# IIT-PAVIS/Acoustic-Image-Generation

Hardware: AMD Instinct MI355X
Metric: train-step images/sec (higher is better)
Workload: dtype f32

## Files before the change

acoustic-image-generation_amd/csrc/conv_halo16_kernel.hpp:

```cpp
#pragma once
#include "igemm_split3_kernel.hpp"

namespace acimg {

struct ConvHaloParams {
    const float* X; int H, W, ldx;
    const char* Wimg; unsigned w_lo_off;
    const float* a_scale; const float* a_shift; int a_relu;
    float* Y; int ldy, nout;
    const float* bias; const float* res; int ldres; const float* mask; int ldmask;
    float* stats; int stats_ld;
    int tiles_x, tiles_y; long tiles;
};

template <typename TR, int TERMS, int CIN, int NOUT, int MODE>
__global__ __launch_bounds__(512, 1) void conv_halo16_kernel(const ConvHaloParams p) {
    typedef typename TR::V8 V8;
    constexpr int TH = TERMS == 1 ? 8 : 4, TW = 32, XH = TH + 2, XWV = TW + 2, XW = 36;
    constexpr int PITCH = CIN * 2 + 16;
    constexpr int XPL = XH * XW * PITCH;
    constexpr int KTOT = 9 * CIN;
    constexpr int WROW = KTOT * 2 + 16;
    constexpr int WPL = NOUT * WROW;
    constexpr int NPL = TERMS == 3 ? 2 : 1;
    constexpr int MT = TERMS == 1 ? 2 : 1;
    constexpr int NT = NOUT / 16;
    constexpr int NXL = (XH * XWV * (CIN / 4) + 511) / 512;
    extern __shared__ __attribute__((aligned(16))) float ch16_smem[];
    char* const xl = reinterpret_cast<char*>(ch16_smem);
    char* const wl = xl + NPL * XPL;
    const int tid = threadIdx.x, lane = tid & 63, wid = tid >> 6;
    const int li = lane & 15, g = lane >> 4;
    const int jrow = TERMS == 1 ? wid : wid >> 1;
    const int mcol0 = TERMS == 1 ? 0 : (wid & 1) * 16;

    for (int i = tid; i < NPL * NOUT * (KTOT / 8); i += 512) {
        const int ch = i % (KTOT / 8), r2 = i / (KTOT / 8);
        const int n = r2 % NOUT, pl = r2 / NOUT;
        const uint4 v = *reinterpret_cast<const uint4*>(p.Wimg + (size_t)pl * p.w_lo_off + ((size_t)n * KTOT + ch * 8) * 2);
        *reinterpret_cast<uint4*>(wl + pl * WPL + n * WROW + ch * 16) = v;
    }

    float4 rx[NXL];
    unsigned okm = 0;
    const float4 asc = p.a_scale ? *reinterpret_cast<const float4*>(p.a_scale + (tid % (CIN / 4)) * 4) : make_float4(1.f, 1.f, 1.f, 1.f);
    const float4 ash = p.a_scale ? *reinterpret_cast<const float4*>(p.a_shift + (tid % (CIN / 4)) * 4) : make_float4(0.f, 0.f, 0.f, 0.f);
    auto load_tile = [&](long tile) {
        okm = 0;
        const int tx = (int)(tile % p.tiles_x);
        const long t2 = tile / p.tiles_x;
        const int ty = (int)(t2 % p.tiles_y);
        const long img = t2 / p.tiles_y;
        const float* xi = p.X + img * p.H * p.W * p.ldx;
#pragma unroll
        for (int k = 0; k < NXL; ++k) {
            const int i = tid + 512 * k;
            const int c4 = i % (CIN / 4), pix = i / (CIN / 4);
            const int row = pix / XWV, col = pix - row * XWV;
            const int iy = ty * TH + row - 1, ix = tx * TW + col - 1;
            float4 v = make_float4(0.f, 0.f, 0.f, 0.f);
            if (row < XH && (unsigned)iy < (unsigned)p.H && (unsigned)ix < (unsigned)p.W) {
                v = *reinterpret_cast<const float4*>(xi + ((long)iy * p.W + ix) * p.ldx + c4 * 4);
                okm |= 1u << k;
            }
            rx[k] = v;
        }
    };
    auto store_tile = [&]() {
#pragma unroll
        for (int k = 0; k < NXL; ++k) {
            const int i = tid + 512 * k;
            const int c4 = i % (CIN / 4), pix = i / (CIN / 4);
            const int row = pix / XWV, col = pix - row * XWV;
            if (row < XH) {
                const int off = (row * XW + col) * PITCH + c4 * 8;
                uint2 hi, lo;
                split4<TR>(p.a_scale && ((okm >> k) & 1u) ? affine_relu4(rx[k], asc, ash, p.a_relu != 0) : rx[k], hi, lo);
                *reinterpret_cast<uint2*>(xl + off) = hi;
                if (TERMS == 3) *reinterpret_cast<uint2*>(xl + XPL + off) = lo;
            }
        }
    };

    f32x4 s1[NT], s2[NT];
#pragma unroll
    for (int n = 0; n < NT; ++n) s1[n] = s2[n] = f32x4{0.f, 0.f, 0.f, 0.f};
    f32x4 bv[NT];
#pragma unroll
    for (int n = 0; n < NT; ++n)
        bv[n] = (MODE == 0 && p.bias) ? *reinterpret_cast<const f32x4*>(p.bias + n * 16 + 4 * g) : f32x4{0.f, 0.f, 0.f, 0.f};

    const int a_base = (jrow * XW + mcol0 + li) * PITCH + g * 16;
    const int b_base = li * WROW + g * 16;

    long tile = blockIdx.x;
    if (tile < p.tiles) load_tile(tile);
    for (; tile < p.tiles; tile += gridDim.x) {
        __syncthreads();
        store_tile();
        __syncthreads();
        const int tx = (int)(tile % p.tiles_x);
        const long t2 = tile / p.tiles_x;
        const int ty = (int)(t2 % p.tiles_y);
        const long img = t2 / p.tiles_y;
        if (tile + gridDim.x < p.tiles) load_tile(tile + gridDim.x);
        f32x4 acc[MT][NT];
#pragma unroll
        for (int m = 0; m < MT; ++m)
#pragma unroll
            for (int n = 0; n < NT; ++n) acc[m][n] = f32x4{0.f, 0.f, 0.f, 0.f};
#pragma unroll
        for (int r = 0; r < 3; ++r)
#pragma unroll
            for (int s_ = 0; s_ < 3; ++s_)
#pragma unroll
                for (int ck = 0; ck < CIN / 32; ++ck) {
                    V8 ah[MT], al[MT], bh[NT], bl[NT];
#pragma unroll
                    for (int m = 0; m < MT; ++m) {
                        const int off = a_base + (r * XW + s_ + 16 * m) * PITCH + ck * 64;
                        ah[m] = *reinterpret_cast<const V8*>(xl + off);
                        if (TERMS == 3) al[m] = *reinterpret_cast<const V8*>(xl + XPL + off);
                    }
#pragma unroll
                    for (int n = 0; n < NT; ++n) {
                        const int off = b_base + n * 16 * WROW + ((r * 3 + s_) * CIN + ck * 32) * 2;
                        bh[n] = *reinterpret_cast<const V8*>(wl + off);
                        if (TERMS == 3) bl[n] = *reinterpret_cast<const V8*>(wl + WPL + off);
                    }
#pragma unroll
                    for (int m = 0; m < MT; ++m)
#pragma unroll
                        for (int n = 0; n < NT; ++n) {
                            if (TERMS == 3) {
                                acc[m][n] = TR::mfma(bl[n], ah[m], acc[m][n]);
                                acc[m][n] = TR::mfma(bh[n], al[m], acc[m][n]);
                            }
                            acc[m][n] = TR::mfma(bh[n], ah[m], acc[m][n]);
                        }
                }
        const int oy = ty * TH + jrow;
#pragma unroll
        for (int m = 0; m < MT; ++m) {
            const int ox = tx * TW + mcol0 + 16 * m + li;
            if (oy < p.H && ox < p.W) {
                const long pix = (img * p.H + oy) * p.W + ox;
#pragma unroll
                for (int n = 0; n < NT; ++n) {
                    if (NOUT == 16 && n * 16 + 4 * g >= p.nout) continue;
                    f32x4 v = acc[m][n] * TR::OUTSCALE + bv[n];
                    if (MODE == 1) {
                        if (p.res) v += *reinterpret_cast<const f32x4*>(p.res + pix * p.ldres + n * 16 + 4 * g);
                        if (p.mask) {
                            const f32x4 k = *reinterpret_cast<const f32x4*>(p.mask + pix * p.ldmask + n * 16 + 4 * g);
#pragma unroll
                            for (int c = 0; c < 4; ++c) v[c] = k[c] > 0.f ? v[c] : 0.f;
                        }
                    } else {
                        s1[n] += v;
                        s2[n] += v * v;
                    }
                    *reinterpret_cast<f32x4*>(p.Y + pix * p.ldy + n * 16 + 4 * g) = v;
                }
            }
        }
    }
    if (MODE == 0 && p.stats) {
        __syncthreads();
        float* red = reinterpret_cast<float*>(xl);
#pragma unroll
        for (int n = 0; n < NT; ++n)
#pragma unroll
            for (int c = 0; c < 4; ++c) {
                const float a = row16_sum(s1[n][c]), b = row16_sum(s2[n][c]);
                if (li == 0) {
                    red[(wid * 2 + 0) * NOUT + n * 16 + 4 * g + c] = a;
                    red[(wid * 2 + 1) * NOUT + n * 16 + 4 * g + c] = b;
                }
            }
        __syncthreads();
        if (tid < 2 * NOUT) {
            const int which = tid / NOUT, n = tid % NOUT;
            float t = 0.f;
#pragma unroll
            for (int w = 0; w < 8; ++w) t += red[(w * 2 + which) * NOUT + n];
            p.stats[((long)blockIdx.x * 2 + which) * p.stats_ld + n] = t;
        }
    }
}

static constexpr int CONV_HALO16_WGS = 256;

}
```

acoustic-image-generation_amd/csrc/igemm.hip:

```cpp
#include "wgrad_split3_kernel.hpp"
#include "wgrad_tap_kernel.hpp"
#include "conv_tap_kernel.hpp"
#include "igemm_split3d_kernel.hpp"
#include "igemm_split3dp_kernel.hpp"
#include "igemm_split3r_kernel.hpp"
#include "igemm_split3h_kernel.hpp"
#include "skinny_kernel.hpp"
#include "wgrad_f32_kernel.hpp"
#include "wgrad_halo_kernel.hpp"
#include "direct_conv_kernel.hpp"
#include "conv_few16_kernel.hpp"
#include "patch2_kernel.hpp"
#include "conv_halo16_kernel.hpp"
#include "conv_aux_kernels.hpp"
#include <cstdlib>
#include <algorithm>
#include <type_traits>

namespace acimg {

static void launch_slab_reduce_wide(const float* slab, int splits, long rows, int ncols, int ld, float* out, const float* slab2,
                                    float* out2, hipStream_t st) {
    const long total = rows * ncols;
    if (total <= 4096) {
// ... 138 lines not shown
            return fail(ACIMG_EINVAL, "igemm: ticket words must be 16-byte aligned");
        const bool handoff = tickets != nullptr && tiles <= ACIMG_TICKET_WORDS && g_cfg.splitk_handoff;
        if (handoff) need = (size_t)p.splits * tiles * c.bm * c.bn * sizeof(float);
        if (ws == nullptr || ws_bytes < need)
            return fail(ACIMG_EWORKSPACE, "igemm: workspace %zu < %zu", ws_bytes, need);
        p.slab = static_cast<float*>(ws);
        if (handoff) p.ts_counters = static_cast<int*>(tickets);
    }
    if (c.bm == 128 && c.bn == 128) launch_cfg<128, 128, 2, 4, 512>(p, nt, cal, grid, st);
    else if (c.bm == 128 && c.bn == 64) launch_cfg<128, 64, 2, 2, 256>(p, nt, cal, grid, st);
    else if (c.bm == 64 && c.bn == 64) launch_cfg<64, 64, 2, 2, 256>(p, nt, cal, grid, st);
    else launch_cfg<256, 16, 4, 1, 256>(p, nt, cal, grid, st);
    int rc = check_launch("igemm");
    if (rc) return rc;
    if (p.splits > 1) {
        if (p.ts_counters == nullptr) {
            const long total = (long)p.M * p.Ngemm;
            hipLaunchKernelGGL(igemm_splitk_reduce_kernel, dim3(cdiv(total, 256)), dim3(256), 0, st,
                               p.slab, p.splits, p.M, p.Ngemm, p.slab_ld, p.e);
            rc = check_launch("igemm_splitk_reduce");
        }
        if (!rc && stats_after) {
            hipLaunchKernelGGL(partial_stats_kernel, dim3(cdiv(p.M, 256)), dim3(256), 0, st, e.Y, e.ldy, p.M,
                               e.Nstore, stats_after, e.stats_ld, 256);
            rc = check_launch("partial_stats");
        }
    }
    return rc;
}

static int pick_wgrad_splits(int M, int KK, int Ngemm, int bmo, int bn) {
    const long tiles = (long)cdiv(KK, bmo) * cdiv(Ngemm, bn);
    long s = (512 + tiles - 1) / tiles;
    const int minpix = g_cfg.wgrad_minpix;
    const long maxs = (M + minpix - 1) / minpix;
    long cap = 128;
    if ((long)KK * Ngemm <= 8192) {
        s = (2048 + tiles - 1) / tiles;
        cap = 2048;
    }
    if (s > maxs) s = maxs;
    if (s > cap) s = cap;
    if (s < 1) s = 1;
    return (int)s;
}
static void wgrad_tile(int Ngemm, int& bmo, int& bn) {
    bmo = 128;
    bn = Ngemm <= 16 ? 16 : (Ngemm <= 32 ? 32 : (Ngemm <= 64 ? 64 : 128));
    if (Ngemm > 64 && cdiv(Ngemm, 64) * 64 < cdiv(Ngemm, 128) * 128) bn = 64;
}
static int wgrad_split3_bn(int Ngemm) {
    return Ngemm > 64 ? 128 : (Ngemm > 32 ? 64 : 32);
}
static bool wgrad_halo16_shape(long M, int KK, int Ngemm) { return Ngemm <= 32 && KK % 9 == 0 && KK <= 9 * 64 && M >= 65536; }
static bool wgrad_tap_shape(int KK, int Ngemm) { return KK % 9 == 0 && KK >= 9 * 64 && Ngemm > 32; }
static size_t wgrad_ws_bytes(int M, int KK, int Ngemm, int ldo) {
    int bmo, bn;
    wgrad_tile(Ngemm, bmo, bn);
    int s = std::max(pick_wgrad_splits(M, KK, Ngemm, bmo, bn), pick_wgrad_splits(M, KK, Ngemm, bmo, wgrad_split3_bn(Ngemm)));
    if (wgrad_halo16_shape(M, KK, Ngemm) && s < (KK <= 9 * 16 ? 512 : 256)) s = KK <= 9 * 16 ? 512 : 256;
    return s > 1 ? (size_t)(s + 1) * ((size_t)KK + 1) * ldo * sizeof(float) : 0;
}

static bool wgrad_halo_ok(const WgradParams& p) {
    return (p.C == 4 || p.C == 8 || p.C == 16) && p.Nld <= 16 && p.Ngemm == p.Nld && p.stride == 1 && p.R <= 3 && p.S <= 3 && (long)p.M >= 65536 && (p.ldx & 3) == 0 && (p.ldg & 3) == 0 &&
           (p.KK + 1 + 15) / 16 <= WH_MAXT && wgrad_halo_lds(p.R, p.S, p.C, p.Nld, p.stride) <= 65536 &&
           g_cfg.wgrad_halo;
}

static bool wgrad_halo16_ok(const WgradParams& p, bool split3) {
    const bool few = p.C < 32;
    return wgrad_halo16_shape(p.M, p.KK, p.Ngemm) && (split3 || few) && p.R == 3 && p.S == 3 && p.stride == 1 && p.pad_t == 1 &&
           p.pad_l == 1 && (p.C == 64 || (p.C <= 32 && p.C % 4 == 0)) && p.Ngemm % 4 == 0 && p.Nld == p.Ngemm && p.OH == p.H &&
           p.OW == p.W && p.ldo >= p.Ngemm && g_cfg.wgrad_halo;
}

static bool wgrad_tap_ok(const WgradParams& p) {
    return wgrad_tap_shape(p.KK, p.Ngemm) && p.R == 3 && p.S == 3 && p.stride == 1 && p.pad_t == 1 && p.pad_l == 1 &&
           p.OH == p.H && p.OW == p.W && p.W % 16 == 0 && p.W >= 32 && p.W <= WT_MAXW && p.KK == 9 * p.C && p.Nld == p.Ngemm &&
           p.Ngemm % 4 == 0 && p.ldo >= p.Ngemm && p.M % (p.H * p.W) == 0 && !p.a_scale && g_cfg.wgrad_halo;
}

struct WgradSlabs {
    size_t need;
    bool fits;
    float *out, *db_rows, *db_out;
};
static WgradSlabs wgrad_slabs(const WgradParams& p, int n, const float* db, void* ws, size_t ws_bytes) {
    WgradSlabs s{};
    s.need = (size_t)n * ((size_t)p.KK + 1) * p.ldo * sizeof(float);
    s.fits = ws != nullptr && ws_bytes >= s.need;
    if (s.fits) {
        s.out = static_cast<float*>(ws);
        s.db_rows = s.out + (size_t)n * p.KK * p.ldo;
        s.db_out = db ? s.db_rows : nullptr;
    }
    return s;
}
static int wgrad_ws_short(const WgradSlabs& s, size_t ws_bytes) {
    return fail(ACIMG_EWORKSPACE, "wgrad: workspace %zu < %zu", ws_bytes, s.need);
}
static int wgrad_reduce(const WgradSlabs& s, int n, const WgradParams& p, float* dw, float* db, bool wide, hipStream_t st) {
    if (wide || n > 32) {
        launch_slab_reduce_wide(s.out, n, (long)p.KK, p.Ngemm, p.ldo, dw, s.db_out, db, st);
    } else {
        const long total = (long)p.KK * p.Ngemm;
        const int nb1 = (int)cdiv(total, 256), nb2 = db ? cdiv(p.Ngemm, 256) : 0;
        hipLaunchKernelGGL(slab_reduce_kernel, dim3(nb1 + nb2), dim3(256), 0, st, s.out, n, (long)p.KK, p.Ngemm, p.ldo, dw, nb1,
                           s.db_rows, db);
    }
    return check_launch("wgrad_reduce");
}

static int launch_wgrad(WgradParams p, float* dw, float* db, void* ws, size_t ws_bytes, hipStream_t st,
                        bool split3 = false, int terms = 3) {
    if ((p.C & 3) || (p.ldx & 3) || (p.ldg & 3) || (p.ldo & 3))
        return fail(ACIMG_EINVAL, "wgrad: C=%d ldx=%d ldg=%d ldo=%d must be multiples of 4", p.C, p.ldx, p.ldg, p.ldo);
    if (!aligned16(p.X) || !aligned16(p.G) || !aligned16(dw))
        return fail(ACIMG_EINVAL, "wgrad: operands must be 16-byte aligned");
    if (p.a_scale && !wgrad_halo16_ok(p, split3))
        return fail(ACIMG_EINVAL, "wgrad: an input affine is only taken by the halo form (3x3 / stride 1 / SAME, <= 32 columns, >= 65536 pixels)");
    if (p.a_scale && (!p.a_shift || !aligned16(p.a_scale) || !aligned16(p.a_shift)))
        return fail(ACIMG_EINVAL, "wgrad: the input affine needs scale and shift, 16-byte aligned");
    int bmo, bn;
    wgrad_tile(p.Ngemm, bmo, bn);
    if (wgrad_halo16_ok(p, split3)) {
        WgradHalo16Params q{};
        q.X = p.X; q.H = p.H; q.W = p.W; q.ldx = p.ldx; q.G = p.G; q.ldg = p.ldg; q.ldo = p.ldo;
        q.creal = p.C; q.nreal = p.Ngemm;
        q.a_scale = p.a_scale; q.a_shift = p.a_shift; q.a_relu = p.a_relu;
        if (p.C < 32) terms = 3;
        const int cpad = p.C == 64 ? 64 : (p.C > 16 ? 32 : 16);
        const int nnt = (cpad == 16 && p.Ngemm <= 16) ? 1 : 2;
        const int th = (terms == 1 || cpad == 16) ? 8 : 4;
        q.tiles_x = cdiv(p.W, 32); q.tiles_y = cdiv(p.H, th);
        q.tiles = (long)(p.M / (p.H * p.W)) * q.tiles_x * q.tiles_y;
        int nb = p.C <= 16 ? 512 : 256;
        if (nb > q.tiles) nb = (int)q.tiles;
        const WgradSlabs sl = wgrad_slabs(p, nb, db, ws, ws_bytes);
        if (sl.fits) {
            q.out = sl.out;
            q.db_out = sl.db_out;
            const int xh = th + 2, planes = terms == 3 ? 2 : 1;
            int lds = planes * (xh * 36 * cpad * 2 + th * 32 * 64);
            if (lds < 4 * 10 * 64 * 16) lds = 4 * 10 * 64 * 16;
#define ACIMG_WH16(Cv, Tv)                                                                                              \
    do {                                                                                                                \
        static bool attr_set = false;                                                                                   \
        if (!attr_set) {                                                                                                \
            (void)hipFuncSetAttribute(reinterpret_cast<const void*>(wgrad_halo16_kernel<Cv, Tv>),                       \
                                      hipFuncAttributeMaxDynamicSharedMemorySize, 2 * (10 * 36 * 64 * 2 + 8 * 32 * 64)); \
            attr_set = true;                                                                                            \
        }                                                                                                               \
        hipLaunchKernelGGL((wgrad_halo16_kernel<Cv, Tv>), dim3(nb), dim3(512), lds, st, q);                             \
    } while (0)
            if (cpad == 64 && terms == 1) ACIMG_WH16(64, 1);
            else if (cpad == 64) ACIMG_WH16(64, 3);
            else if (cpad == 32 && terms == 1) ACIMG_WH16(32, 1);
            else if (cpad == 32) ACIMG_WH16(32, 3);
            else if (nnt == 2) ACIMG_WH16(16, 3);
            else {
                static bool attr16 = false;
                if (!attr16) {
                    (void)hipFuncSetAttribute(reinterpret_cast<const void*>(wgrad_halo16_kernel<16, 3, 1>),
                                              hipFuncAttributeMaxDynamicSharedMemorySize, 65536);
                    attr16 = true;
                }
                hipLaunchKernelGGL((wgrad_halo16_kernel<16, 3, 1>), dim3(nb), dim3(512), lds, st, q);
            }
#undef ACIMG_WH16
            int rc = check_launch("wgrad_halo16");
            return rc ? rc : wgrad_reduce(sl, nb, p, dw, db, true, st);
        }
    }
    if (p.a_scale) return fail(ACIMG_EWORKSPACE, "wgrad: workspace too small for the halo form, which the input affine needs");
    if (wgrad_halo_ok(p)) {
        WgradHaloParams q{};
        q.X = p.X; q.H = p.H; q.W = p.W; q.C = p.C; q.ldx = p.ldx;
        q.G = p.G; q.OH = p.OH; q.OW = p.OW; q.Kp = p.Nld; q.ldg = p.ldg;
        q.R = p.R; q.S = p.S; q.stride = p.stride; q.pad_t = p.pad_t; q.pad_l = p.pad_l;
        q.XH = (WH_TH - 1) * p.stride + p.R; q.XW = (WH_TW - 1) * p.stride + p.S;
        q.tiles_x = cdiv(p.OW, WH_TW); q.tiles_y = cdiv(p.OH, WH_TH);
        q.tiles = (long)(p.M / (p.OH * p.OW)) * q.tiles_x * q.tiles_y;
        q.KK = p.KK; q.ldo = p.ldo;
// ... 238 lines not shown
    if ((Ko & 3) || (Kin & 3)) return fail(ACIMG_EINVAL, "%s: channel counts must be multiples of 4", what);
    float* wc = static_cast<float*>(ws);
    hipLaunchKernelGGL(subpixel_weights_kernel, dim3(cdiv((long)rows * ncol, 256)), dim3(256), 0, st, w, R, S, Ko, Kin, ldw, U, V, wc,
                       rows * ncol);
    int rc = check_launch("subpixel_weights");
    if (rc) return rc;
    IgemmParams p{};
    p.A = A; p.H = aH; p.W = aW; p.C = Kin; p.lda = lda; p.OH = AH; p.OW = AW;
    p.R = U; p.S = V; p.stride = 1; p.pad_t = U - 1; p.pad_l = V - 1;
    p.M = N * AH * AW;
    p.rowrun = (V > 1 && lda == Kin) ? 1 : 0;
    p.B = wc; p.ldb = ncol; p.Nld = ncol; p.Ngemm = ncol; p.tap_stride = 0; p.flip = 0;
    p.e.Y = Y; p.e.ldy = ldy; p.e.M = p.M; p.e.Nstore = ncol; p.e.bias = bias; p.e.act = act;
    p.e.res = res; p.e.ldres = ldres; p.e.mask = mask; p.e.ldmask = ldmask;
    p.e.scatter = 2; p.e.Ko = Ko; p.e.Sq = 2; p.e.sc = 2; p.e.YH = YH; p.e.YW = YW; p.e.AH = AH; p.e.AW = AW;
    p.e.oy0 = oy0; p.e.ox0 = ox0;
    return launch_igemm(p, false, static_cast<char*>(ws) + wcb, ws_bytes - wcb, tickets, st);
}

static bool dgrad_is_patch(const AcimgConvDesc* d) {
    return d->stride > 1 && d->stride == d->R && d->stride == d->S && !d->pad_t && !d->pad_l &&
           d->OH * d->stride == d->H && d->OW * d->stride == d->W;
}
static size_t dilated_bytes(int N, int H, int W, int C, int s) {
    return ((size_t)N * ((H - 1) * s + 1) * ((W - 1) * s + 1) * C * 4 + 255) & ~(size_t)255;
}

static bool dgrad_halo16_narrow_shape(const AcimgConvDesc* d) {
    return d->R == 3 && d->S == 3 && d->stride == 1 && d->pad_t == 1 && d->pad_l == 1 && d->OH == d->H && d->OW == d->W &&
           d->K == 32 && d->C <= 16 && (d->C & 3) == 0 && (long)d->N * d->H * d->W >= 65536 && g_cfg.wgrad_halo;
}
static constexpr size_t DGRAD_HALO16_NARROW_WS = 2 * 16 * 288 * 2;
struct Split3Cfg { int bm, bn; };
static Split3Cfg pick_split3(int M, int K, bool allow32 = false) {
    if (K <= 32 && allow32) return {128, 32};
    if (K <= 64) return {128, 64};
    if (g_cfg.split3_tile_bm) {
        return {g_cfg.split3_tile_bm, g_cfg.split3_tile_bn};
    }
    if ((long)cdiv(M, 128) * cdiv(K, 128) < 200) return {64, 128};
    return {128, 128};
}

static bool conv_halo16_fwd_shape(const AcimgConvDesc* d) {
    return d->R == 3 && d->S == 3 && d->stride == 1 && d->pad_t == 1 && d->pad_l == 1 && d->OH == d->H && d->OW == d->W &&
           (d->C == 32 || d->C == 64) && d->K == 32 && (long)d->N * d->H * d->W >= 65536 && d->act == ACIMG_ACT_NONE &&
           g_cfg.wgrad_halo;
}
static bool conv_halo16_dgrad_shape(const AcimgConvDesc* d) {
    return d->R == 3 && d->S == 3 && d->stride == 1 && d->pad_t == 1 && d->pad_l == 1 && d->OH == d->H && d->OW == d->W &&
           (d->C == 32 || d->C == 64) && d->K == 32 && (long)d->N * d->H * d->W >= 65536 && g_cfg.wgrad_halo;
}

template <typename TR, int TERMS, int CIN, int NOUT, int MODE>
static int launch_conv_halo16(ConvHaloParams q, int N, hipStream_t st) {
    constexpr int TH = TERMS == 1 ? 8 : 4, NPL = TERMS == 3 ? 2 : 1;
    constexpr int lds = NPL * ((TH + 2) * 36 * (CIN * 2 + 16) + NOUT * (9 * CIN * 2 + 16));
    static_assert(lds <= 160 * 1024 && 8 * 2 * NOUT * 4 <= lds, "LDS budget");
    q.tiles_x = cdiv(q.W, 32); q.tiles_y = cdiv(q.H, TH);
    q.tiles = (long)N * q.tiles_x * q.tiles_y;
    if (!q.nout) q.nout = NOUT;
    static bool attr_set = false;
    if (!attr_set) {
        (void)hipFuncSetAttribute(reinterpret_cast<const void*>(conv_halo16_kernel<TR, TERMS, CIN, NOUT, MODE>),
                                  hipFuncAttributeMaxDynamicSharedMemorySize, lds);
        attr_set = true;
    }
    hipLaunchKernelGGL((conv_halo16_kernel<TR, TERMS, CIN, NOUT, MODE>), dim3(CONV_HALO16_WGS), dim3(512), lds, st, q);
    return check_launch("conv_halo16");
}

static int dgrad_halo16_narrow(const AcimgConvDesc* d, const float* gy, int ldgy, const float* w, float* dx, int lddx,
                               const float* residual, int ldres, const float* mask, int ldmask, void* ws, hipStream_t st) {
    FewParams f{};
    f.w = w; f.ldw = d->ldw; f.wrows = d->C; f.cin = d->K; f.mode = 1; f.nout = d->C;
    hipLaunchKernelGGL((few16_prepare_kernel<SplitBF16>), dim3(cdiv(16 * 288, 256)), dim3(256), 0, st, f, 32, 16,
                       static_cast<__bf16*>(ws));
    ConvHaloParams q{};
    q.X = gy; q.H = d->H; q.W = d->W; q.ldx = ldgy; q.Wimg = static_cast<const char*>(ws); q.w_lo_off = 16 * 288 * 2;
    q.Y = dx; q.ldy = lddx; q.nout = d->C; q.res = residual; q.ldres = ldres; q.mask = mask; q.ldmask = ldmask;
    return launch_conv_halo16<SplitBF16, 3, 32, 16, 1>(q, d->N, st);
}

enum TrunkKind { TRUNK_ONE_TILE = 0, TRUNK_PERSISTENT = 1, TRUNK_RING = 2, TRUNK_HALO = 3 };
struct TrunkPick {
    TrunkKind kind;
    int bm, bn;
    int stats_rows;
    bool big_out;
};

static constexpr int HALO_NB = 18;
static bool halo_applies(const AcimgConvDesc* d, int terms, const Split3Cfg& c) {
    if (terms != 3 || d->R != 3 || d->S != 3 || d->stride != 1 || d->pad_t != 1 || d->pad_l != 1 || d->OH != d->H ||
        d->OW != d->W || d->C % 32)
        return false;
    if (c.bm != 128 || c.bn != 128) return false;
    return ((d->W + 16) >> 4) + 8 + (d->W >> 4) + 1 <= HALO_NB;
}

static TrunkPick pick_trunk(const AcimgConvDesc* d, int terms, bool two_pass) {
    const int M = d->N * d->OH * d->OW;
    const Split3Cfg c = pick_split3(M, d->K);
    const bool t128 = c.bm == 128 && c.bn == 128;
    TrunkPick t{TRUNK_ONE_TILE, c.bm, c.bn, 0, (long)M * d->ldy * 4 >= (1L << 31)};
    if (two_pass) t.kind = TRUNK_PERSISTENT;
    else if (g_cfg.trunk_halo == 2 && halo_applies(d, terms, c)) t.kind = TRUNK_HALO;
    int ring_rows = 0;
    if (!two_pass && t.kind != TRUNK_HALO && !t.big_out && g_cfg.trunk_ring && terms == 3 && t128) {
        const long t128s = (long)cdiv(M, 128) * cdiv(d->K, 128);
        const int kiters = d->R * d->S * (d->C / 32);
        const long t256 = (long)cdiv(M, 256) * cdiv(d->K, 128);
        if (g_cfg.trunk_ring == 1) ring_rows = (t128s > 256 && t128s <= 300 && kiters >= 64) ? 128 : 0;
        else if (g_cfg.trunk_ring_bm) ring_rows = g_cfg.trunk_ring_bm;
        else ring_rows = t256 >= 500 ? 256 : 128;
    }
    if (ring_rows) {
        t.kind = TRUNK_RING;
        t.bm = ring_rows;
    }
    const long tiles = (long)cdiv(M, c.bm) * cdiv(d->K, c.bn);
    if (t.kind == TRUNK_ONE_TILE && !t.big_out && t128 && (g_cfg.trunk_persistent == 2 || (g_cfg.trunk_persistent == 1 && tiles >= 512)))
        t.kind = TRUNK_PERSISTENT;
    t.stats_rows = cdiv(M, t.bm);
    return t;
}

static size_t split3_rowmajor_bytes(const AcimgConvDesc* d) { return (size_t)2 * d->ldw * d->R * d->S * d->C * 2; }
static size_t split3_brick_bytes(const AcimgConvDesc* d) {
    return d->C % 32 ? 0 : (size_t)cdiv(d->ldw, 128) * (d->R * d->S * d->C / 32) * 2 * 8192;
}

template <typename TR, int TERMS = 3>
static int launch_split3(IgemmParams& p, hipStream_t st) {
// ... 334 lines not shown
}

using namespace acimg;

extern "C" {

int acimg_conv2d_stats_rows(const AcimgConvDesc* d) {
    if (few16_fwd_shape(d)) return FEW16_WGS;
    return cdiv((long)d->N * d->OH * d->OW, stats_block_rows(d));
}

int acimg_conv2d_fwd_tiling(const AcimgConvDesc* d, int* out) {
    if (!d || !out) return fail(ACIMG_EINVAL, "conv2d_fwd_tiling: null argument");
    const int M = d->N * d->OH * d->OW;
    TileCfg c = pick_cfg(M, d->K);
    out[0] = c.bm;
    out[1] = c.bn;
    out[2] = pick_splits(M, d->K, c, fwd_kiters(d));
    return ACIMG_OK;
}

int acimg_config_default(AcimgConfig* c) {
    if (!c) return fail(ACIMG_EINVAL, "config_default: null");
    *c = DEFAULT_CFG;
    return ACIMG_OK;
}

int acimg_configure(const AcimgConfig* c) {
    if (!c) return fail(ACIMG_EINVAL, "configure: null");
    if (c->splitk_cut < 0 || c->splitk_target < 1 || c->wgrad_minpix < 1 || c->tail_s < 0)
        return fail(ACIMG_EINVAL, "configure: negative / zero tuning value");
    if (c->trunk_persistent < 0 || c->trunk_persistent > 2) return fail(ACIMG_EINVAL, "configure: trunk_persistent is 0, 1 or 2");
    if (c->trunk_dma_pos < 0 || c->trunk_dma_pos > 1) return fail(ACIMG_EINVAL, "configure: trunk_dma_pos is 0 or 1");
    if (c->trunk_stagger < 0 || c->trunk_stagger > 100) return fail(ACIMG_EINVAL, "configure: trunk_stagger is a percentage");
    if (c->trunk_bk != 0 && c->trunk_bk != 32)
        return fail(ACIMG_EINVAL, "configure: trunk_bk must be 0 or 32 (the 64-deep K step was measured slower and removed)");
    if (c->trunk_ring < 0 || c->trunk_ring > 2) return fail(ACIMG_EINVAL, "configure: trunk_ring is 0, 1 or 2");
    if (c->trunk_ring_bm != 0 && c->trunk_ring_bm != 128 && c->trunk_ring_bm != 256)
        return fail(ACIMG_EINVAL, "configure: trunk_ring_bm must be 0 (per shape), 128 or 256");
    if (c->trunk_halo < 0 || c->trunk_halo > 2) return fail(ACIMG_EINVAL, "configure: trunk_halo is 0, 1 or 2");
    if (c->split3_tile_bm || c->split3_tile_bn) {
        const int bm = c->split3_tile_bm, bn = c->split3_tile_bn;
        if (!((bm == 128 && bn == 128) || (bm == 64 && bn == 128) || (bm == 128 && bn == 64)))
            return fail(ACIMG_EINVAL, "configure: split3 tile %dx%d is not an instantiated tile", bm, bn);
    }
    g_cfg = *c;
    return ACIMG_OK;
}

size_t acimg_conv2d_fwd_workspace(const AcimgConvDesc* d) {
    const size_t a = igemm_ws_bytes(d->N * d->OH * d->OW, d->K, fwd_kiters(d));
    const size_t b = direct_shape(d->C, d->K) ? direct_ws_bytes(d->R, d->S, d->C, (d->K + 7) & ~7) : 0;
    const size_t c = skinny_fwd_ws_bytes(d);
    const size_t f = few16_fwd_shape(d) ? few16_ws_bytes(d->C, d->K) : 0;
    return std::max(std::max(a, f), std::max(b, c));
}

int acimg_conv2d_fwd(const AcimgConvDesc* d, const float* x, const float* w, const float* bias,
                     float* y, const float* in_scale, const float* in_shift, int in_relu,
                     float* stats, void* ws, size_t ws_bytes, void* tickets, void* stream) {
    int rc = check_desc(d, "conv2d_fwd");
    if (rc) return rc;
    if (d->ldw < d->K) return fail(ACIMG_EINVAL, "conv2d_fwd: ldw < K");
    if (skinny_shape(d) && !in_scale && !in_shift && !in_relu && !stats && ws && ws_bytes >= skinny_fwd_ws_bytes(d) && aligned16(x) &&
        aligned16(w) && aligned16(y) && aligned16(ws) && (!bias || aligned16(bias)) && (d->ldw & 3) == 0 && (d->ldx & 3) == 0 &&
        (d->ldy & 3) == 0) {
        SkinnyParams q{};
        q.W = w; q.X = x; q.out = y; q.bias = bias; q.act = d->act; q.part = static_cast<float*>(ws);
        q.M = d->N; q.C = d->C; q.N = d->K; q.ldw = d->ldw; q.ldx = d->ldx; q.ldo = d->ldy;
        q.slabs = cdiv(d->C, SKINNY_KS);
        const dim3 grid(q.slabs, cdiv(d->K, 64));
        const int mb = cdiv(d->N, 16);
        if (mb == 1) hipLaunchKernelGGL(skinny_fwd_kernel<1>, grid, dim3(64), 0, (hipStream_t)stream, q);
        else if (mb == 2) hipLaunchKernelGGL(skinny_fwd_kernel<2>, grid, dim3(64), 0, (hipStream_t)stream, q);
        else if (mb == 3) hipLaunchKernelGGL(skinny_fwd_kernel<3>, grid, dim3(64), 0, (hipStream_t)stream, q);
        else hipLaunchKernelGGL(skinny_fwd_kernel<4>, grid, dim3(64), 0, (hipStream_t)stream, q);
        rc = check_launch("conv2d_fwd (skinny)");
        if (rc) return rc;
        hipLaunchKernelGGL(skinny_fwd_reduce_kernel, dim3(cdiv(d->N * (d->K / 4), 256)), dim3(256), 0, (hipStream_t)stream, q);
        return check_launch("conv2d_fwd (skinny reduce)");
    }
    if (few16_fwd_shape(d)) {
        if ((in_scale != nullptr) != (in_shift != nullptr) || (in_relu && !in_scale) || !aligned16(x) || !aligned16(y) || (d->ldy & 3) ||
            d->ldy < d->K || (bias && !aligned16(bias)) || (in_scale && (!aligned16(in_scale) || !aligned16(in_shift))))
            return fail(ACIMG_EINVAL, "conv2d_fwd: few-channel MFMA shape with half an input affine or unaligned operands");
        FewParams q{};
        q.a_scale = in_scale; q.a_shift = in_shift; q.a_relu = in_relu;
        q.X = x; q.H = d->H; q.W = d->W; q.ldx = d->ldx; q.Y = y; q.ldy = d->ldy; q.nout = d->K; q.bias = bias;
        q.Hin = q.SH = d->H; q.Win = q.SW = d->W; q.dil = 1; q.pad_t = 1; q.pad_l = 1;
        q.stats = stats; q.stats_ld = d->ldw;
        q.w = w; q.ldw = d->ldw; q.wrows = d->C; q.cin = d->C; q.mode = 0;
        return dispatch_few16<0>(q, d->N, d->C, d->K, ws, ws_bytes, (hipStream_t)stream);
    }
    if (direct_ok(d->C, d->K, d->ldy, 0, y, bias, nullptr, in_scale != nullptr, nullptr) &&
        (long)d->N * d->OH * d->OW >= 65536) {
        DirectParams q{};
        q.x = x; q.ldx = d->ldx; q.H = d->H; q.W = d->W; q.C = d->C;
        q.y = y; q.ldy = d->ldy; q.OH = d->OH; q.OW = d->OW; q.K = d->K;
        q.R = d->R; q.S = d->S; q.stride = d->stride; q.pad_t = d->pad_t; q.pad_l = d->pad_l;
        q.w = w; q.ldw = d->ldw; q.mode = 0; q.wrows = d->C; q.bias = bias; q.act = d->act;
        q.M = (long)d->N * d->OH * d->OW;
        const bool fuse_stats = stats && stats_block_rows(d) == 256 && d->act == ACIMG_ACT_NONE;
        if (fuse_stats) { q.stats = stats; q.stats_ld = d->ldw; }
        rc = launch_direct(q, ws, ws_bytes, (hipStream_t)stream);
        if (!rc && stats && !fuse_stats) {
            hipLaunchKernelGGL(partial_stats_kernel, dim3(acimg_conv2d_stats_rows(d)), dim3(256), 0, (hipStream_t)stream,
                               y, d->ldy, (int)q.M, d->K, stats, d->ldw, stats_block_rows(d));
            rc = check_launch("partial_stats");
        }
        return rc;
    }
    IgemmParams p = fwd_view(d);
    p.A = x; p.rowrun = (d->S > 1 && d->ldx == d->C) ? 1 : 0;
    p.a_scale = in_scale; p.a_shift = in_shift; p.a_relu = in_relu;
    p.B = w; p.ldb = d->ldw;
    p.e.Y = y; p.e.bias = bias; p.e.stats = stats;
    return launch_igemm(p, false, ws, ws_bytes, tickets, (hipStream_t)stream);
}

size_t acimg_conv2d_dgrad_workspace(const AcimgConvDesc* d) {
    if (dgrad_halo16_narrow_shape(d)) return DGRAD_HALO16_NARROW_WS + 256;
    if (dgrad_is_patch(d)) return igemm_ws_bytes(d->N * d->OH * d->OW, d->R * d->S * d->C, cdiv(up4(d->K), 32));
    const int ca = up4(d->K);
    if (subpixel_ok(d->stride, d->C, ca))
        return subpixel_ws_bytes(d->N, d->H, d->W, -d->pad_t, -d->pad_l, d->R, d->S, ca, d->C);
    if (d->stride > 1)
        return dilated_bytes(d->N, d->OH, d->OW, ca, d->stride) +
               igemm_ws_bytes(d->N * d->H * d->W, d->C, d->R * d->S * cdiv(ca, 32)) +
               igemm_ws_bytes(d->N * d->H * d->W, d->C, d->R * cdiv(d->S * ca, 32)) +
               (direct_shape(ca, d->C) ? std::max(direct_ws_bytes(d->R, d->S, ca, (d->C + 7) & ~7), few16_ws_bytes(ca, d->C)) : 0);
    return igemm_ws_bytes(d->N * d->H * d->W, d->C, d->R * d->S * cdiv(ca, 32)) +
           igemm_ws_bytes(d->N * d->H * d->W, d->C, d->R * cdiv(d->S * ca, 32)) +
           (direct_shape(ca, d->C) ? std::max(direct_ws_bytes(d->R, d->S, ca, (d->C + 7) & ~7), few16_ws_bytes(ca, d->C)) : 0);
}

int acimg_conv2d_dgrad(const AcimgConvDesc* d, const float* gy, int ldgy, const float* w,
                       float* dx, int lddx, const float* residual, int ldres, const float* mask,
                       int ldmask, void* ws, size_t ws_bytes, void* tickets, void* stream) {
    int rc = check_desc(d, "conv2d_dgrad");
    if (rc) return rc;
    const int ca = up4(d->K);
    if (ca > ldgy || ca > d->ldw || (ldgy & 3)) return fail(ACIMG_EINVAL, "conv2d_dgrad: padded K=%d exceeds ldgy=%d/ldw=%d", ca, ldgy, d->ldw);
    if (skinny_shape(d) && aligned16(gy) && aligned16(w) && (d->ldw & 3) == 0) {
        SkinnyParams q{};
        q.W = w; q.G = gy; q.out = dx; q.res = residual; q.mask = mask;
        q.M = d->N; q.C = d->C; q.N = ca;
        q.ldw = d->ldw; q.ldg = ldgy; q.ldo = lddx > 0 ? lddx : d->ldx; q.ldres = ldres; q.ldmask = ldmask;
        if (q.ldo < d->C) return fail(ACIMG_EINVAL, "conv2d_dgrad: lddx < C");
        const dim3 grid(cdiv(cdiv(d->C, 16), 4));
        const int mb = cdiv(d->N, 16);
        if (mb == 1) hipLaunchKernelGGL(skinny_dgrad_kernel<1>, grid, dim3(256), 0, (hipStream_t)stream, q);
        else if (mb == 2) hipLaunchKernelGGL(skinny_dgrad_kernel<2>, grid, dim3(256), 0, (hipStream_t)stream, q);
        else if (mb == 3) hipLaunchKernelGGL(skinny_dgrad_kernel<3>, grid, dim3(256), 0, (hipStream_t)stream, q);
        else hipLaunchKernelGGL(skinny_dgrad_kernel<4>, grid, dim3(256), 0, (hipStream_t)stream, q);
        return check_launch("conv2d_dgrad (skinny)");
    }
    if (lddx <= 0) lddx = d->ldx;
    if (lddx < d->C) return fail(ACIMG_EINVAL, "conv2d_dgrad: lddx < C");
    if (subpixel_ok(d->stride, d->C, ca) && !dgrad_is_patch(d))
        return launch_subpixel(gy, d->N, d->OH, d->OW, ca, ldgy, w, d->R, d->S, d->ldw, d->C, dx, lddx, d->H, d->W, -d->pad_t,
                               -d->pad_l, nullptr, residual, ldres, mask, ldmask, ACIMG_ACT_NONE, ws, ws_bytes, tickets,
                               (hipStream_t)stream, "conv2d_dgrad");
    if (dgrad_halo16_narrow_shape(d) && aligned16(gy) && aligned16(dx) && (lddx & 3) == 0 && ws && aligned16(ws) &&
        ws_bytes >= DGRAD_HALO16_NARROW_WS && (!residual || ((ldres & 3) == 0 && aligned16(residual))) &&
        (!mask || ((ldmask & 3) == 0 && aligned16(mask))))
        return dgrad_halo16_narrow(d, gy, ldgy, w, dx, lddx, residual, ldres, mask, ldmask, ws, (hipStream_t)stream);
    if (few16_dgrad_shape(d) && !subpixel_ok(d->stride, d->C, ca) && !mask && aligned16(gy) && aligned16(dx) && (lddx & 3) == 0 &&
        ws && aligned16(ws) && ws_bytes >= few16_ws_bytes(ca, d->C) && (!residual || ((ldres & 3) == 0 && aligned16(residual)))) {
        FewParams q{};
        q.X = gy; q.ldx = ldgy; q.SH = d->OH; q.SW = d->OW; q.dil = d->stride;
        q.Hin = (d->OH - 1) * d->stride + 1; q.Win = (d->OW - 1) * d->stride + 1;
        q.pad_t = 2 - d->pad_t; q.pad_l = 2 - d->pad_l;
        q.H = d->H; q.W = d->W; q.Y = dx; q.ldy = lddx; q.nout = d->C;
        q.res = residual; q.ldres = ldres;
        q.w = w; q.ldw = d->ldw; q.wrows = d->C; q.cin = d->K; q.mode = 1;
        return dispatch_few16<1>(q, d->N, ca, d->C, ws, ws_bytes, (hipStream_t)stream);
    }
    if (d->stride > 1 && !dgrad_is_patch(d)) {
        const size_t db = dilated_bytes(d->N, d->OH, d->OW, ca, d->stride);
        if (ws_bytes < db || !ws) return fail(ACIMG_EWORKSPACE, "conv2d_dgrad: workspace too small for the dilated gradient");
        const int OH1 = (d->OH - 1) * d->stride + 1, OW1 = (d->OW - 1) * d->stride + 1;
        const long opix = (long)d->N * OH1 * OW1;
        if (opix * ca >= (1L << 31)) return fail(ACIMG_EINVAL, "conv2d_dgrad: dilated gradient exceeds 2^31 elements");
        hipLaunchKernelGGL(dilate2d_kernel, dim3(cdiv(opix * (ca / 4), 256)), dim3(256), 0, (hipStream_t)stream, gy, ldgy,
                           static_cast<float*>(ws), opix, d->OH, d->OW, OH1, OW1, ca, d->stride);
        rc = check_launch("dilate2d");
        if (rc) return rc;
        AcimgConvDesc d1 = *d;
        d1.stride = 1; d1.OH = OH1; d1.OW = OW1;
        return acimg_conv2d_dgrad(&d1, static_cast<const float*>(ws), ca, w, dx, lddx, residual, ldres, mask, ldmask,
                                  static_cast<char*>(ws) + db, ws_bytes - db, tickets, stream);
    }
    if (d->stride == 1 && direct_ok(ca, d->C, lddx, ldres, dx, nullptr, residual, false, mask) &&
        (long)d->N * d->H * d->W >= 65536) {
        DirectParams q{};
        q.x = gy; q.ldx = ldgy; q.H = d->OH; q.W = d->OW; q.C = ca;
        q.y = dx; q.ldy = lddx; q.OH = d->H; q.OW = d->W; q.K = d->C;
        q.R = d->R; q.S = d->S; q.stride = 1; q.pad_t = d->R - 1 - d->pad_t; q.pad_l = d->S - 1 - d->pad_l;
        q.w = w; q.ldw = d->ldw; q.mode = 1; q.wrows = d->C; q.act = ACIMG_ACT_NONE;
        q.res = residual; q.ldres = ldres;
        q.M = (long)d->N * d->H * d->W;
        return launch_direct(q, ws, ws_bytes, (hipStream_t)stream);
    }
    IgemmParams p{};
    if (d->stride == 1) {
        p = flipped_view(d, ca, ldgy);
        p.rowrun = (d->S > 1 && ldgy == ca) ? 1 : 0;
        p.tap_stride = (long)d->C * d->ldw; p.flip = 1;
    } else {
        p.H = d->OH; p.W = d->OW; p.C = ca; p.lda = ldgy; p.OH = d->OH; p.OW = d->OW;
        p.R = 1; p.S = 1; p.stride = 1;
        p.M = d->N * d->OH * d->OW;
        p.Ngemm = d->R * d->S * d->C;
        p.e.M = p.M; p.e.Nstore = p.Ngemm; p.e.act = ACIMG_ACT_NONE;
        p.e.scatter = 1; p.e.Ko = d->C; p.e.Sq = d->S; p.e.sc = d->stride;
        p.e.YH = d->H; p.e.YW = d->W; p.e.AH = d->OH; p.e.AW = d->OW;
    }
    p.A = gy; p.B = w; p.ldb = d->ldw;
    p.e.Y = dx; p.e.ldy = lddx; p.e.res = residual; p.e.ldres = ldres; p.e.mask = mask; p.e.ldmask = ldmask;
// ... 443 lines not shown
```

Measured before the change: 5328.

## Route 64↔12 and 12→128 edge convolutions through split-precision halo MFMA kernel

```diff
diff --git a/acoustic-image-generation_amd/csrc/conv_halo16_kernel.hpp b/acoustic-image-generation_amd/csrc/conv_halo16_kernel.hpp
--- a/acoustic-image-generation_amd/csrc/conv_halo16_kernel.hpp
+++ b/acoustic-image-generation_amd/csrc/conv_halo16_kernel.hpp
@@ -8,12 +8,30 @@
     const char* Wimg; unsigned w_lo_off;
     const float* a_scale; const float* a_shift; int a_relu;
     float* Y; int ldy, nout;
+    int act;
     const float* bias; const float* res; int ldres; const float* mask; int ldmask;
     float* stats; int stats_ld;
     int tiles_x, tiles_y; long tiles;
 };
 
-template <typename TR, int TERMS, int CIN, int NOUT, int MODE>
+template <typename TR>
+__global__ __launch_bounds__(256) void conv_halo16_prepare_kernel(const float* w, int ldw, int wrows, int cin, int nout, int mode,
+                                                                  int CIN, int NOUT, typename TR::T* img) {
+    typedef typename TR::T T;
+    const int KTOT = 9 * CIN;
+    const int i = blockIdx.x * 256 + threadIdx.x;
+    if (i >= NOUT * KTOT) return;
+    const int row = i / KTOT, k = i - row * KTOT;
+    const int tap = k / CIN, c = k - tap * CIN;
+    float v = 0.f;
+    if (row < nout && c < cin) v = mode == 0 ? w[((long)tap * wrows + c) * ldw + row] : w[((long)(8 - tap) * wrows + row) * ldw + c];
+    v *= TR::WSCALE;
+    const T h = (T)v;
+    img[i] = h;
+    img[(size_t)NOUT * KTOT + i] = (T)(v - (float)h);
+}
+
+template <typename TR, int TERMS, int CIN, int NOUT, int MODE, int CLOAD = CIN>
 __global__ __launch_bounds__(512, 1) void conv_halo16_kernel(const ConvHaloParams p) {
     typedef typename TR::V8 V8;
     constexpr int TH = TERMS == 1 ? 8 : 4, TW = 32, XH = TH + 2, XWV = TW + 2, XW = 36;
@@ -25,7 +43,8 @@
     constexpr int NPL = TERMS == 3 ? 2 : 1;
     constexpr int MT = TERMS == 1 ? 2 : 1;
     constexpr int NT = NOUT / 16;
-    constexpr int NXL = (XH * XWV * (CIN / 4) + 511) / 512;
+    constexpr int NXL = (XH * XWV * (CLOAD / 4) + 511) / 512;
+    static_assert(CLOAD % 4 == 0 && CLOAD <= CIN, "channels read");
     extern __shared__ __attribute__((aligned(16))) float ch16_smem[];
     char* const xl = reinterpret_cast<char*>(ch16_smem);
     char* const wl = xl + NPL * XPL;
@@ -34,17 +53,18 @@
     const int jrow = TERMS == 1 ? wid : wid >> 1;
     const int mcol0 = TERMS == 1 ? 0 : (wid & 1) * 16;
 
+    const int cb = blockIdx.y * NOUT;
     for (int i = tid; i < NPL * NOUT * (KTOT / 8); i += 512) {
         const int ch = i % (KTOT / 8), r2 = i / (KTOT / 8);
         const int n = r2 % NOUT, pl = r2 / NOUT;
-        const uint4 v = *reinterpret_cast<const uint4*>(p.Wimg + (size_t)pl * p.w_lo_off + ((size_t)n * KTOT + ch * 8) * 2);
+        const uint4 v = *reinterpret_cast<const uint4*>(p.Wimg + (size_t)pl * p.w_lo_off + ((size_t)(cb + n) * KTOT + ch * 8) * 2);
         *reinterpret_cast<uint4*>(wl + pl * WPL + n * WROW + ch * 16) = v;
     }
 
     float4 rx[NXL];
     unsigned okm = 0;
-    const float4 asc = p.a_scale ? *reinterpret_cast<const float4*>(p.a_scale + (tid % (CIN / 4)) * 4) : make_float4(1.f, 1.f, 1.f, 1.f);
-    const float4 ash = p.a_scale ? *reinterpret_cast<const float4*>(p.a_shift + (tid % (CIN / 4)) * 4) : make_float4(0.f, 0.f, 0.f, 0.f);
+    const float4 asc = p.a_scale ? *reinterpret_cast<const float4*>(p.a_scale + (tid % (CLOAD / 4)) * 4) : make_float4(1.f, 1.f, 1.f, 1.f);
+    const float4 ash = p.a_scale ? *reinterpret_cast<const float4*>(p.a_shift + (tid % (CLOAD / 4)) * 4) : make_float4(0.f, 0.f, 0.f, 0.f);
     auto load_tile = [&](long tile) {
         okm = 0;
         const int tx = (int)(tile % p.tiles_x);
@@ -55,7 +75,7 @@
 #pragma unroll
         for (int k = 0; k < NXL; ++k) {
             const int i = tid + 512 * k;
-            const int c4 = i % (CIN / 4), pix = i / (CIN / 4);
+            const int c4 = i % (CLOAD / 4), pix = i / (CLOAD / 4);
             const int row = pix / XWV, col = pix - row * XWV;
             const int iy = ty * TH + row - 1, ix = tx * TW + col - 1;
             float4 v = make_float4(0.f, 0.f, 0.f, 0.f);
@@ -70,7 +90,7 @@
 #pragma unroll
         for (int k = 0; k < NXL; ++k) {
             const int i = tid + 512 * k;
-            const int c4 = i % (CIN / 4), pix = i / (CIN / 4);
+            const int c4 = i % (CLOAD / 4), pix = i / (CLOAD / 4);
             const int row = pix / XWV, col = pix - row * XWV;
             if (row < XH) {
                 const int off = (row * XW + col) * PITCH + c4 * 8;
@@ -82,13 +102,17 @@
         }
     };
 
+    if (CLOAD < CIN) {
+        for (int i = tid; i < NPL * XPL / 16; i += 512) *reinterpret_cast<uint4*>(xl + i * 16) = make_uint4(0u, 0u, 0u, 0u);
+    }
+
     f32x4 s1[NT], s2[NT];
 #pragma unroll
     for (int n = 0; n < NT; ++n) s1[n] = s2[n] = f32x4{0.f, 0.f, 0.f, 0.f};
     f32x4 bv[NT];
 #pragma unroll
     for (int n = 0; n < NT; ++n)
-        bv[n] = (MODE == 0 && p.bias) ? *reinterpret_cast<const f32x4*>(p.bias + n * 16 + 4 * g) : f32x4{0.f, 0.f, 0.f, 0.f};
+        bv[n] = (MODE == 0 && p.bias && n * 16 + 4 * g < p.nout) ? *reinterpret_cast<const f32x4*>(p.bias + cb + n * 16 + 4 * g) : f32x4{0.f, 0.f, 0.f, 0.f};
 
     const int a_base = (jrow * XW + mcol0 + li) * PITCH + g * 16;
     const int b_base = li * WROW + g * 16;
@@ -150,17 +174,21 @@
                     if (NOUT == 16 && n * 16 + 4 * g >= p.nout) continue;
                     f32x4 v = acc[m][n] * TR::OUTSCALE + bv[n];
                     if (MODE == 1) {
-                        if (p.res) v += *reinterpret_cast<const f32x4*>(p.res + pix * p.ldres + n * 16 + 4 * g);
+                        if (p.res) v += *reinterpret_cast<const f32x4*>(p.res + pix * p.ldres + cb + n * 16 + 4 * g);
                         if (p.mask) {
-                            const f32x4 k = *reinterpret_cast<const f32x4*>(p.mask + pix * p.ldmask + n * 16 + 4 * g);
+                            const f32x4 k = *reinterpret_cast<const f32x4*>(p.mask + pix * p.ldmask + cb + n * 16 + 4 * g);
 #pragma unroll
                             for (int c = 0; c < 4; ++c) v[c] = k[c] > 0.f ? v[c] : 0.f;
                         }
                     } else {
+                        if (p.act != ACIMG_ACT_NONE) {
+#pragma unroll
+                            for (int c = 0; c < 4; ++c) v[c] = epi_act(v[c], p.act);
+                        }
                         s1[n] += v;
                         s2[n] += v * v;
                     }
-                    *reinterpret_cast<f32x4*>(p.Y + pix * p.ldy + n * 16 + 4 * g) = v;
+                    *reinterpret_cast<f32x4*>(p.Y + pix * p.ldy + cb + n * 16 + 4 * g) = v;
                 }
             }
         }
diff --git a/acoustic-image-generation_amd/csrc/igemm.hip b/acoustic-image-generation_amd/csrc/igemm.hip
--- a/acoustic-image-generation_amd/csrc/igemm.hip
+++ b/acoustic-image-generation_amd/csrc/igemm.hip
@@ -214,7 +214,12 @@
 static int wgrad_split3_bn(int Ngemm) {
     return Ngemm > 64 ? 128 : (Ngemm > 32 ? 64 : 32);
 }
-static bool wgrad_halo16_shape(long M, int KK, int Ngemm) { return Ngemm <= 32 && KK % 9 == 0 && KK <= 9 * 64 && M >= 65536; }
+static constexpr long EDGE_MIN_PIXELS = 49152;
+static bool edge_pixels(long pixels) { return pixels >= EDGE_MIN_PIXELS; }
+static bool wgrad_edge_shape(long M, int KK, int Ngemm) { return KK == 9 * 64 && Ngemm == 12 && edge_pixels(M); }
+static bool wgrad_halo16_shape(long M, int KK, int Ngemm) {
+    return Ngemm <= 32 && KK % 9 == 0 && KK <= 9 * 64 && (M >= 65536 || wgrad_edge_shape(M, KK, Ngemm));
+}
 static bool wgrad_tap_shape(int KK, int Ngemm) { return KK % 9 == 0 && KK >= 9 * 64 && Ngemm > 32; }
 static size_t wgrad_ws_bytes(int M, int KK, int Ngemm, int ldo) {
     int bmo, bn;
@@ -231,7 +236,7 @@
 }
 
 static bool wgrad_halo16_ok(const WgradParams& p, bool split3) {
-    const bool few = p.C < 32;
+    const bool few = p.C < 32 || (p.C == 64 && wgrad_edge_shape(p.M, p.KK, p.Ngemm));
     return wgrad_halo16_shape(p.M, p.KK, p.Ngemm) && (split3 || few) && p.R == 3 && p.S == 3 && p.stride == 1 && p.pad_t == 1 &&
            p.pad_l == 1 && (p.C == 64 || (p.C <= 32 && p.C % 4 == 0)) && p.Ngemm % 4 == 0 && p.Nld == p.Ngemm && p.OH == p.H &&
            p.OW == p.W && p.ldo >= p.Ngemm && g_cfg.wgrad_halo;
@@ -291,7 +296,7 @@
         q.X = p.X; q.H = p.H; q.W = p.W; q.ldx = p.ldx; q.G = p.G; q.ldg = p.ldg; q.ldo = p.ldo;
         q.creal = p.C; q.nreal = p.Ngemm;
         q.a_scale = p.a_scale; q.a_shift = p.a_shift; q.a_relu = p.a_relu;
-        if (p.C < 32) terms = 3;
+        if (p.C < 32 || !split3) terms = 3;
         const int cpad = p.C == 64 ? 64 : (p.C > 16 ? 32 : 16);
         const int nnt = (cpad == 16 && p.Ngemm <= 16) ? 1 : 2;
         const int th = (terms == 1 || cpad == 16) ? 8 : 4;
@@ -636,7 +641,7 @@
            (d->C == 32 || d->C == 64) && d->K == 32 && (long)d->N * d->H * d->W >= 65536 && g_cfg.wgrad_halo;
 }
 
-template <typename TR, int TERMS, int CIN, int NOUT, int MODE>
+template <typename TR, int TERMS, int CIN, int NOUT, int MODE, int CLOAD = CIN, int NB = 1>
 static int launch_conv_halo16(ConvHaloParams q, int N, hipStream_t st) {
     constexpr int TH = TERMS == 1 ? 8 : 4, NPL = TERMS == 3 ? 2 : 1;
     constexpr int lds = NPL * ((TH + 2) * 36 * (CIN * 2 + 16) + NOUT * (9 * CIN * 2 + 16));
@@ -644,13 +649,14 @@
     q.tiles_x = cdiv(q.W, 32); q.tiles_y = cdiv(q.H, TH);
     q.tiles = (long)N * q.tiles_x * q.tiles_y;
     if (!q.nout) q.nout = NOUT;
+    if (NB > 1 && q.stats) return fail(ACIMG_EINVAL, "conv_halo16: no statistics over several column blocks");
     static bool attr_set = false;
     if (!attr_set) {
-        (void)hipFuncSetAttribute(reinterpret_cast<const void*>(conv_halo16_kernel<TR, TERMS, CIN, NOUT, MODE>),
+        (void)hipFuncSetAttribute(reinterpret_cast<const void*>(conv_halo16_kernel<TR, TERMS, CIN, NOUT, MODE, CLOAD>),
                                   hipFuncAttributeMaxDynamicSharedMemorySize, lds);
         attr_set = true;
     }
-    hipLaunchKernelGGL((conv_halo16_kernel<TR, TERMS, CIN, NOUT, MODE>), dim3(CONV_HALO16_WGS), dim3(512), lds, st, q);
+    hipLaunchKernelGGL((conv_halo16_kernel<TR, TERMS, CIN, NOUT, MODE, CLOAD>), dim3((NB > 1 && 2 * lds <= 160 * 1024 ? 2 : 1) * CONV_HALO16_WGS / NB, NB), dim3(512), lds, st, q);
     return check_launch("conv_halo16");
 }
 
@@ -664,6 +670,42 @@
     q.X = gy; q.H = d->H; q.W = d->W; q.ldx = ldgy; q.Wimg = static_cast<const char*>(ws); q.w_lo_off = 16 * 288 * 2;
     q.Y = dx; q.ldy = lddx; q.nout = d->C; q.res = residual; q.ldres = ldres; q.mask = mask; q.ldmask = ldmask;
     return launch_conv_halo16<SplitBF16, 3, 32, 16, 1>(q, d->N, st);
+}
+
+static bool edge_geometry(const AcimgConvDesc* d) {
+    return d->R == 3 && d->S == 3 && d->stride == 1 && d->pad_t == 1 && d->pad_l == 1 && d->OH == d->H && d->OW == d->W &&
+           edge_pixels((long)d->N * d->H * d->W) && g_cfg.wgrad_halo;
+}
+static bool edge_fwd_shape(const AcimgConvDesc* d) { return edge_geometry(d) && d->C == 64 && d->K == 12 && d->ldx >= 64; }
+static constexpr size_t EDGE_FWD_WS = 2 * 16 * 576 * 2;
+static int edge_fwd(const AcimgConvDesc* d, const float* x, const float* w, const float* bias, float* y, void* ws, hipStream_t st) {
+    hipLaunchKernelGGL((conv_halo16_prepare_kernel<SplitF16>), dim3(cdiv(16 * 576, 256)), dim3(256), 0, st, w, d->ldw, d->C, d->C,
+                       d->K, 0, 64, 16, static_cast<_Float16*>(ws));
+    ConvHaloParams q{};
+    q.X = x; q.H = d->H; q.W = d->W; q.ldx = d->ldx; q.Wimg = static_cast<const char*>(ws); q.w_lo_off = 16 * 576 * 2;
+    q.Y = y; q.ldy = d->ldy; q.nout = d->K; q.bias = bias; q.act = d->act;
+    return launch_conv_halo16<SplitF16, 3, 64, 16, 0>(q, d->N, st);
+}
+static bool edge_fwd12_shape(const AcimgConvDesc* d) { return edge_geometry(d) && d->C == 12 && d->K == 128 && d->ldx >= 12; }
+static constexpr size_t EDGE_FWD12_WS = 2 * 128 * 288 * 2;
+static int edge_fwd12(const AcimgConvDesc* d, const float* x, const float* w, const float* bias, float* y, void* ws, hipStream_t st) {
+    hipLaunchKernelGGL((conv_halo16_prepare_kernel<SplitF16>), dim3(cdiv(128 * 288, 256)), dim3(256), 0, st, w, d->ldw, d->C, d->C,
+                       d->K, 0, 32, 128, static_cast<_Float16*>(ws));
+    ConvHaloParams q{};
+    q.X = x; q.H = d->H; q.W = d->W; q.ldx = d->ldx; q.Wimg = static_cast<const char*>(ws); q.w_lo_off = 128 * 288 * 2;
+    q.Y = y; q.ldy = d->ldy; q.bias = bias; q.act = d->act;
+    return launch_conv_halo16<SplitF16, 3, 32, 32, 0, 12, 4>(q, d->N, st);
+}
+static bool edge_dgrad_shape(const AcimgConvDesc* d) { return edge_geometry(d) && d->C == 64 && d->K == 12; }
+static constexpr size_t EDGE_DGRAD_WS = 2 * 64 * 288 * 2;
+static int edge_dgrad(const AcimgConvDesc* d, const float* gy, int ldgy, const float* w, float* dx, int lddx, const float* residual,
+                      int ldres, const float* mask, int ldmask, void* ws, hipStream_t st) {
+    hipLaunchKernelGGL((conv_halo16_prepare_kernel<SplitBF16>), dim3(cdiv(64 * 288, 256)), dim3(256), 0, st, w, d->ldw, d->C, d->K,
+                       d->C, 1, 32, 64, static_cast<__bf16*>(ws));
+    ConvHaloParams q{};
+    q.X = gy; q.H = d->H; q.W = d->W; q.ldx = ldgy; q.Wimg = static_cast<const char*>(ws); q.w_lo_off = 64 * 288 * 2;
+    q.Y = dx; q.ldy = lddx; q.res = residual; q.ldres = ldres; q.mask = mask; q.ldmask = ldmask;
+    return launch_conv_halo16<SplitBF16, 3, 32, 32, 1, 12, 2>(q, d->N, st);
 }
 
 enum TrunkKind { TRUNK_ONE_TILE = 0, TRUNK_PERSISTENT = 1, TRUNK_RING = 2, TRUNK_HALO = 3 };
@@ -1104,7 +1146,7 @@
     const size_t a = igemm_ws_bytes(d->N * d->OH * d->OW, d->K, fwd_kiters(d));
     const size_t b = direct_shape(d->C, d->K) ? direct_ws_bytes(d->R, d->S, d->C, (d->K + 7) & ~7) : 0;
     const size_t c = skinny_fwd_ws_bytes(d);
-    const size_t f = few16_fwd_shape(d) ? few16_ws_bytes(d->C, d->K) : 0;
+    const size_t f = few16_fwd_shape(d) ? few16_ws_bytes(d->C, d->K) : (edge_fwd_shape(d) ? EDGE_FWD_WS : (edge_fwd12_shape(d) ? EDGE_FWD12_WS : 0));
     return std::max(std::max(a, f), std::max(b, c));
 }
 
@@ -1144,6 +1186,18 @@
         q.w = w; q.ldw = d->ldw; q.wrows = d->C; q.cin = d->C; q.mode = 0;
         return dispatch_few16<0>(q, d->N, d->C, d->K, ws, ws_bytes, (hipStream_t)stream);
     }
+    if (edge_fwd_shape(d) && !stats && !in_scale && !in_shift && !in_relu) {
+        if (!aligned16(x) || !aligned16(y) || (d->ldy & 3) || d->ldy < d->K || (bias && !aligned16(bias)))
+            return fail(ACIMG_EINVAL, "conv2d_fwd: the 64 -> 12 halo form needs 16-byte aligned operands and ldy %% 4 == 0");
+        if (!ws || ws_bytes < EDGE_FWD_WS || !aligned16(ws)) return fail(ACIMG_EWORKSPACE, "conv2d_fwd: workspace %zu < %zu", ws_bytes, EDGE_FWD_WS);
+        return edge_fwd(d, x, w, bias, y, ws, (hipStream_t)stream);
+    }
+    if (edge_fwd12_shape(d) && !stats && !in_scale && !in_shift && !in_relu) {
+        if (!aligned16(x) || !aligned16(y) || (d->ldy & 3) || d->ldy < d->K || (bias && !aligned16(bias)))
+            return fail(ACIMG_EINVAL, "conv2d_fwd: the 12 -> 128 halo form needs 16-byte aligned operands and ldy %% 4 == 0");
+        if (!ws || ws_bytes < EDGE_FWD12_WS || !aligned16(ws)) return fail(ACIMG_EWORKSPACE, "conv2d_fwd: workspace %zu < %zu", ws_bytes, EDGE_FWD12_WS);
+        return edge_fwd12(d, x, w, bias, y, ws, (hipStream_t)stream);
+    }
     if (direct_ok(d->C, d->K, d->ldy, 0, y, bias, nullptr, in_scale != nullptr, nullptr) &&
         (long)d->N * d->OH * d->OW >= 65536) {
         DirectParams q{};
@@ -1181,6 +1235,7 @@
                igemm_ws_bytes(d->N * d->H * d->W, d->C, d->R * d->S * cdiv(ca, 32)) +
                igemm_ws_bytes(d->N * d->H * d->W, d->C, d->R * cdiv(d->S * ca, 32)) +
                (direct_shape(ca, d->C) ? std::max(direct_ws_bytes(d->R, d->S, ca, (d->C + 7) & ~7), few16_ws_bytes(ca, d->C)) : 0);
+    if (edge_dgrad_shape(d)) return EDGE_DGRAD_WS + 256;
     return igemm_ws_bytes(d->N * d->H * d->W, d->C, d->R * d->S * cdiv(ca, 32)) +
            igemm_ws_bytes(d->N * d->H * d->W, d->C, d->R * cdiv(d->S * ca, 32)) +
            (direct_shape(ca, d->C) ? std::max(direct_ws_bytes(d->R, d->S, ca, (d->C + 7) & ~7), few16_ws_bytes(ca, d->C)) : 0);
@@ -1217,6 +1272,13 @@
         ws_bytes >= DGRAD_HALO16_NARROW_WS && (!residual || ((ldres & 3) == 0 && aligned16(residual))) &&
         (!mask || ((ldmask & 3) == 0 && aligned16(mask))))
         return dgrad_halo16_narrow(d, gy, ldgy, w, dx, lddx, residual, ldres, mask, ldmask, ws, (hipStream_t)stream);
+    if (edge_dgrad_shape(d)) {
+        if (!aligned16(gy) || !aligned16(dx) || (lddx & 3) || (residual && ((ldres & 3) || !aligned16(residual))) ||
+            (mask && ((ldmask & 3) || !aligned16(mask))))
+            return fail(ACIMG_EINVAL, "conv2d_dgrad: the 12 -> 64 halo form needs 16-byte aligned operands and pitches %% 4 == 0");
+        if (!ws || ws_bytes < EDGE_DGRAD_WS || !aligned16(ws)) return fail(ACIMG_EWORKSPACE, "conv2d_dgrad: workspace %zu < %zu", ws_bytes, EDGE_DGRAD_WS);
+        return edge_dgrad(d, gy, ldgy, w, dx, lddx, residual, ldres, mask, ldmask, ws, (hipStream_t)stream);
+    }
     if (few16_dgrad_shape(d) && !subpixel_ok(d->stride, d->C, ca) && !mask && aligned16(gy) && aligned16(dx) && (lddx & 3) == 0 &&
         ws && aligned16(ws) && ws_bytes >= few16_ws_bytes(ca, d->C) && (!residual || ((ldres & 3) == 0 && aligned16(residual)))) {
         FewParams q{};
```

Result: no change. 5348, median of 6 (+0.4%).
